# traveller59/spconv

Measured on AMD Instinct MI355X. Metric: active-voxels/sec fwd+bwd, 3x3x3 SubMConv3d C=64, ~100k voxels/scene, higher is better.
Workload: dtype f16; 1 GPU; SubMConv3d 3x3x3 C=64->64 f16, 100000 uniform voxels/scene in 1600x1280x40 (BASELINE configs[1]), 8 distinct scenes per GPU visited round-robin, rulebook reused via indice_key; voxels_per_gpu=100000, launch=hipgraph, steps_per_replay=8, scenes_rotated=8, mask_sort=False, prewarm_steps=0, parallelism=dp1, ranks_seen=1, tree=unknown

## Files before the change

spconv_amd/csrc/igemm_bwd.h:

```cpp
#pragma once
#include "igemm_v4.h"

namespace spx {
namespace {

constexpr int kWT = 64;

constexpr int kW2MaxG = 1024;
constexpr int kW2J = 128;
constexpr int kW2Rec = 8;
constexpr int kXcds = 8;


__host__ __device__ inline int plan2_wg(int w) { return 8 + kW2Rec * w; }
__host__ __device__ inline int plan2_kf(int G) { return 8 + kW2Rec * G; }
__host__ __device__ inline int plan2_seg(int G, int kv) { return 8 + kW2Rec * G + kv + 1; }
__host__ __device__ inline int plan2_red(int G, int kv) {
  return (plan2_seg(G, kv) + 3 * (G + kv) + 3) & ~3;
}

__device__ __forceinline__ int wtr_x(int row) { return ((row >> 1) & 1) | (((row >> 3) & 1) << 1); }
__device__ __forceinline__ int wtr_slot(int row, int sl) {
  return row * 128 + ((((sl >> 1) ^ wtr_x(row)) << 5) | ((sl & 1) << 4));
}

typedef short s16x4 __attribute__((ext_vector_type(4)));

__device__ __forceinline__ uint4 wtr_frag(const char *stage, int row0, int lrow, int gran) {
  const int r = row0 + (lrow >> 2);
  const char *a0 = stage + r * 128 + ((gran ^ wtr_x(r)) << 5) + ((lrow & 3) << 3);
  const int r1 = r + 4;
  const char *a1 = stage + r1 * 128 + ((gran ^ wtr_x(r1)) << 5) + ((lrow & 3) << 3);
  typedef __attribute__((address_space(3))) s16x4 lds_s16x4;
  const s16x4 lo = __builtin_amdgcn_ds_read_tr16_b64_v4i16(
      (lds_s16x4 *)(__attribute__((address_space(3))) char *)a0);
  const s16x4 hi = __builtin_amdgcn_ds_read_tr16_b64_v4i16(
      (lds_s16x4 *)(__attribute__((address_space(3))) char *)a1);
  const uint2 l2 = __builtin_bit_cast(uint2, lo), h2 = __builtin_bit_cast(uint2, hi);
  return make_uint4(l2.x, l2.y, h2.x, h2.y);
}

template <bool BF16, int STAGES, int SL = 8>
__device__ __forceinline__ void wgrad_tr_body(const Wgrad2Params &p, int block) {
  extern __shared__ __attribute__((aligned(16))) char smem[];
  constexpr int TILE_B = kW2J * 128;
  constexpr int RQ = SL / 2;
  constexpr int RSTEP = 2 * kW2J / SL;
  constexpr int RA = RQ < 2 ? 2 : RQ;
  const int tid = threadIdx.x, lane = tid & 63, wave = tid >> 6;
  const int lrow = lane & 15, lgrp = lane >> 4;
  const int wk = wave >> 1, wc = wave & 1;
  const int ntile = p.tiles_k * p.tiles_c;
  const int wb = block / ntile, tile = block - wb * ntile;
  const int w = p.xcd_order ? p.plan2[plan2_wg(wb) + 5] : wb;
  const int kk0 = (tile / p.tiles_c) * kWT, c0 = (tile % p.tiles_c) * kWT;
  const int32_t *__restrict__ rec = p.plan2 + plan2_wg(w);
  const int32_t *__restrict__ segs = p.plan2 + plan2_seg(p.G, p.kv);
  const int seg_lo = rec[0], nseg = rec[1];
  const bool live = kk0 + wk * 32 < p.K && c0 + wc * 32 < p.C;
  SPX_STAMP(0);

  const uint32_t rowD = static_cast<uint32_t>(p.K) * 2u, rowF = static_cast<uint32_t>(p.C) * 2u;
  const __amdgpu_buffer_rsrc_t rD = make_rsrc(p.dout, static_cast<uint32_t>(p.n_out) * rowD);
  const __amdgpu_buffer_rsrc_t rF = make_rsrc(p.feat, static_cast<uint32_t>(p.n_in) * rowF);
  const uint32_t list_bytes = (static_cast<uint32_t>(p.kv) + 1u) * static_cast<uint32_t>(p.n_in) * 4u;
  const uint32_t out_list = static_cast<uint32_t>(p.kv) * static_cast<uint32_t>(p.n_in) * 4u;

  const int slot = tid & (SL - 1), r0 = tid / SL;
  const uint32_t dcol = kk0 + slot * 8 < p.K ? static_cast<uint32_t>(kk0 + slot * 8) * 2u : kOob;
  const uint32_t fcol = c0 + slot * 8 < p.C ? static_cast<uint32_t>(c0 + slot * 8) * 2u : kOob;
  constexpr int W_ROWS = 64 / SL;
  const int wl_idx = lane & 31;
  const int wl_row = (64 * wave) / SL + (wl_idx % W_ROWS) + RSTEP * (wl_idx / W_ROWS);
  const uint32_t wl_list = (lane >> 5) ? out_list : 0u;
  const int rsub = lane / SL;
  int lds_w[RA];
#pragma unroll
  for (int q = 0; q < RQ; ++q) lds_w[q] = wtr_slot(r0 + RSTEP * q, slot);
  if constexpr (SL < 8) {
    for (int o = tid * 16; o < STAGES * 2 * TILE_B; o += kThreads * 16)
      *reinterpret_cast<u32x4 *>(smem + o) = u32x4{0u, 0u, 0u, 0u};
    __syncthreads();
  }

  for (int si = 0; si < nseg; ++si) {
    int k, begin, end;
    if (si == 0) {
      k = rec[2];
      begin = rec[3];
      end = rec[4];
    } else {
      k = segs[3 * (seg_lo + si)];
      begin = segs[3 * (seg_lo + si) + 1];
      end = segs[3 * (seg_lo + si) + 2];
    }
    const bool identity = p.subm && k == p.kv / 2;
    const __amdgpu_buffer_rsrc_t rW = make_rsrc(p.native + static_cast<size_t>(k) * p.n_in, list_bytes);

    f32x4 acc[2][2];
#pragma unroll
    for (int a = 0; a < 2; ++a)
#pragma unroll
      for (int b = 0; b < 2; ++b) acc[a][b] = f32x4{0.f, 0.f, 0.f, 0.f};

    uint32_t wd = 0;
    u32x4 dv[RA], fv[RA];
    auto load_words = [&](int base) __attribute__((always_inline)) {
      const int j = base + wl_row;
      if (identity) {
        wd = static_cast<uint32_t>(j);
      } else {
        const uint32_t vo = j < end ? static_cast<uint32_t>(j) * 4u + wl_list : kOob;
        wd = __builtin_amdgcn_raw_buffer_load_b32(rW, vo, 0, SPX_AUX_TABLE);
      }
    };
    auto load_rows = [&](int base) __attribute__((always_inline)) {
#pragma unroll
      for (int q = 0; q < RQ; ++q) {
        const uint32_t iq = static_cast<uint32_t>(
            __builtin_amdgcn_ds_bpermute((q * W_ROWS + rsub) * 4, static_cast<int>(wd)));
        const uint32_t oq = static_cast<uint32_t>(
            __builtin_amdgcn_ds_bpermute((32 + q * W_ROWS + rsub) * 4, static_cast<int>(wd)));
        const bool ok = base + r0 + RSTEP * q < end;
        dv[q] = __builtin_amdgcn_raw_buffer_load_b128(rD, ok ? (oq * rowD + dcol) | (dcol & kOob) : kOob, 0, 0);
        fv[q] = __builtin_amdgcn_raw_buffer_load_b128(rF, ok ? (iq * rowF + fcol) | (fcol & kOob) : kOob, 0, 0);
      }
    };
    load_words(begin);
    load_rows(begin);
    load_words(begin + kW2J);
    if (si == 0) SPX_STAMP(1);
    int stage = 0;
    for (int base = begin; base < end; base += kW2J, stage ^= (STAGES - 1)) {
      char *sD = smem + stage * (2 * TILE_B);
      char *sF = sD + TILE_B;
      if (STAGES == 1) __syncthreads();
#pragma unroll
      for (int q = 0; q < RQ; ++q) {
        *reinterpret_cast<u32x4 *>(sD + lds_w[q]) = dv[q];
        *reinterpret_cast<u32x4 *>(sF + lds_w[q]) = fv[q];
      }
      __syncthreads();
      load_rows(base + kW2J);
      load_words(base + 2 * kW2J);
      if (live)
#pragma unroll
      for (int ks = 0; ks < kW2J / 32; ++ks) {
        const int row0 = ks * 32 + lgrp * 8;
        uint4 fa[2], fb[2];
#pragma unroll
        for (int a = 0; a < 2; ++a) fa[a] = wtr_frag(sD, row0, lrow, wk * 2 + a);
#pragma unroll
        for (int b = 0; b < 2; ++b) fb[b] = wtr_frag(sF, row0, lrow, wc * 2 + b);
#pragma unroll
        for (int a = 0; a < 2; ++a)
#pragma unroll
          for (int b = 0; b < 2; ++b) acc[a][b] = mfma16<BF16>(fa[a], fb[b], acc[a][b]);
      }
    }
    if (si == nseg - 1) SPX_STAMP(4);
    float *dst = p.partial + (static_cast<size_t>(seg_lo + si) * ntile + tile) * (kWT * kWT);
#pragma unroll
    for (int a = 0; a < 2; ++a)
#pragma unroll
      for (int b = 0; b < 2; ++b)
#pragma unroll
        for (int e = 0; e < 4; ++e) {
          const int kk = wk * 32 + a * 16 + lgrp * 4 + e;
          const int c = wc * 32 + b * 16 + lrow;
          if (SPX_AUX_OUT) __builtin_nontemporal_store(acc[a][b][e], &dst[kk * kWT + c]);
          else dst[kk * kWT + c] = acc[a][b][e];
        }
    __syncthreads();
  }
  SPX_STAMP(6);
#ifdef SPX_TIMELINE
  asm volatile("s_waitcnt vmcnt(0)" ::: "memory");
  SPX_STAMP(7);
#endif
}

constexpr int kW3J = 64;
constexpr int kW3Stride = 80;

__device__ __forceinline__ void wgrad_f32_body(const Wgrad2Params &p, int block) {
  extern __shared__ __attribute__((aligned(16))) char smem[];
  float *sD = reinterpret_cast<float *>(smem);
  float *sF = sD + kW3J * kW3Stride;
  const int tid = threadIdx.x, lane = tid & 63, wave = tid >> 6;
  const int lrow = lane & 15, lgrp = lane >> 4;
  const int wk = wave >> 1, wc = wave & 1;
  const int ntile = p.tiles_k * p.tiles_c;
  const int w = block / ntile, tile = block - w * ntile;
  const int kk0 = (tile / p.tiles_c) * kWT, c0 = (tile % p.tiles_c) * kWT;
  const int32_t *__restrict__ rec = p.plan2 + plan2_wg(w);
  const int32_t *__restrict__ segs = p.plan2 + plan2_seg(p.G, p.kv);
  const int seg_lo = rec[0], nseg = rec[1];
  const uint32_t rowD = static_cast<uint32_t>(p.K) * 4u, rowF = static_cast<uint32_t>(p.C) * 4u;
  const __amdgpu_buffer_rsrc_t rD = make_rsrc(p.dout, static_cast<uint32_t>(p.n_out) * rowD);
  const __amdgpu_buffer_rsrc_t rF = make_rsrc(p.feat, static_cast<uint32_t>(p.n_in) * rowF);
  const uint32_t list_bytes = static_cast<uint32_t>(p.n_in) * 4u;
  const int slot = tid & 15, r0 = tid >> 4;
  const uint32_t dcol = kk0 + slot * 4 < p.K ? static_cast<uint32_t>(kk0 + slot * 4) * 4u : kOob;
  const uint32_t fcol = c0 + slot * 4 < p.C ? static_cast<uint32_t>(c0 + slot * 4) * 4u : kOob;

  for (int si = 0; si < nseg; ++si) {
    int k, begin, end;
    if (si == 0) {
      k = rec[2];
      begin = rec[3];
      end = rec[4];
    } else {
      k = segs[3 * (seg_lo + si)];
      begin = segs[3 * (seg_lo + si) + 1];
      end = segs[3 * (seg_lo + si) + 2];
    }
    const bool identity = p.subm && k == p.kv / 2;
    const __amdgpu_buffer_rsrc_t rIn =
        make_rsrc(p.native + static_cast<size_t>(k) * p.n_in, list_bytes);
    const __amdgpu_buffer_rsrc_t rOut =
        make_rsrc(p.native + static_cast<size_t>(p.kv + k) * p.n_in, list_bytes);
    f32x4 acc[2][2];
#pragma unroll
    for (int a = 0; a < 2; ++a)
#pragma unroll
      for (int b = 0; b < 2; ++b) acc[a][b] = f32x4{0.f, 0.f, 0.f, 0.f};
    u32x4 dv[4], fv[4];
    auto load_rows = [&](int base) __attribute__((always_inline)) {
#pragma unroll
      for (int q = 0; q < 4; ++q) {
        const int j = base + r0 + 16 * q;
        const bool ok = j < end;
        uint32_t ii = static_cast<uint32_t>(j), oi = static_cast<uint32_t>(j);
        if (!identity) {
          const uint32_t vo = ok ? static_cast<uint32_t>(j) * 4u : kOob;
          ii = __builtin_amdgcn_raw_buffer_load_b32(rIn, vo, 0, 0);
          oi = __builtin_amdgcn_raw_buffer_load_b32(rOut, vo, 0, 0);
        }
        dv[q] = __builtin_amdgcn_raw_buffer_load_b128(rD, ok ? (oi * rowD + dcol) | (dcol & kOob) : kOob, 0, 0);
        fv[q] = __builtin_amdgcn_raw_buffer_load_b128(rF, ok ? (ii * rowF + fcol) | (fcol & kOob) : kOob, 0, 0);
      }
    };
    load_rows(begin);
    for (int base = begin; base < end; base += kW3J) {
      __syncthreads();
#pragma unroll
      for (int q = 0; q < 4; ++q) {
        *reinterpret_cast<u32x4 *>(sD + (r0 + 16 * q) * kW3Stride + slot * 4) = dv[q];
        *reinterpret_cast<u32x4 *>(sF + (r0 + 16 * q) * kW3Stride + slot * 4) = fv[q];
      }
      __syncthreads();
      load_rows(base + kW3J);
#pragma unroll 4
      for (int ks = 0; ks < kW3J / 4; ++ks) {
        const int row = (ks * 4 + lgrp) * kW3Stride;
        float fa[2], fb[2];
#pragma unroll
        for (int a = 0; a < 2; ++a) fa[a] = sD[row + wk * 32 + a * 16 + lrow];
#pragma unroll
        for (int b = 0; b < 2; ++b) fb[b] = sF[row + wc * 32 + b * 16 + lrow];
#pragma unroll
        for (int a = 0; a < 2; ++a)
#pragma unroll
          for (int b = 0; b < 2; ++b)
            acc[a][b] = __builtin_amdgcn_mfma_f32_16x16x4f32(fa[a], fb[b], acc[a][b], 0, 0, 0);
      }
    }
    float *dst = p.partial + (static_cast<size_t>(seg_lo + si) * ntile + tile) * (kWT * kWT);
#pragma unroll
    for (int a = 0; a < 2; ++a)
#pragma unroll
      for (int b = 0; b < 2; ++b)
#pragma unroll
        for (int e = 0; e < 4; ++e) {
          const int kk = wk * 32 + a * 16 + lgrp * 4 + e;
          const int c = wc * 32 + b * 16 + lrow;
          if (SPX_AUX_OUT) __builtin_nontemporal_store(acc[a][b][e], &dst[kk * kWT + c]);
          else dst[kk * kWT + c] = acc[a][b][e];
        }
    __syncthreads();
  }
}

template <int COUT, int MB, int DT, int NKS = 2, int PK = 1>
__global__ void __launch_bounds__(kThreads, COUT <= 64 ? 4 : 2)
igemm_bwd_kernel(const void *argA, const void *argB, const uint32_t *arg_mask,
                 const int32_t *arg_argsort, const int32_t *arg_pair, int n_dst, int n_src, int CIN,
                 int kv, int identity_k, int b_reverse, GemmRest rest, int n_dgrad, Wgrad2Params wp) {
  const int nw = n_dgrad < 0 ? ~n_dgrad : 0;
  const int b = static_cast<int>(blockIdx.x);
  const bool is_dgrad = n_dgrad < 0 ? b >= nw : b < n_dgrad;
  if (is_dgrad) {
    GemmParams p;
    unpack_gemm_args(p, argA, argB, arg_mask, arg_argsort, arg_pair, n_dst, n_src, CIN, kv,
                     identity_k, b_reverse, rest);
    p.xcd_rot = (rest.dbg & 0x100) ? 0 : (nw & 7);
    p.app_budget = kAppBudget;
    igemm_v4_body<COUT, MB, DT, true, NKS, PK>(p, n_dgrad < 0 ? b - nw : b);
  } else {
    if constexpr (DT == 3) wgrad_f32_body(wp, n_dgrad < 0 ? b : b - n_dgrad);
    else wgrad_tr_body<DT == 1, 1>(wp, n_dgrad < 0 ? b : b - n_dgrad);
  }
}

template <int COUT, int MB, int DT = 0>
constexpr size_t bwd_smem_bytes() {
  const size_t a = v4_smem_bytes<COUT, MB>();
  const size_t b = DT == 3 ? 2 * static_cast<size_t>(kW3J) * kW3Stride * sizeof(float)
                           : 2 * static_cast<size_t>(kW2J) * 128;
  return a > b ? a : b;
}

template <int COUT, int MB, int DT>
int launch_bwd(const GemmParams &p, const Wgrad2Params &q, int n_wgrad_blocks, hipStream_t s) {
  const int napp = p.cls ? layout_app_tiles(p.n_dst, 64 * MB) : 0;
  const int n_dgrad = div_up(p.n_dst, 64 * MB) + napp;
  GemmRest rr = rest_of(p);
  rr.napp = p.cls ? napp : -1;
  constexpr int wgrad_first = 1;
  GemmParams pl = p;
  pl.lpt = p.tile_order && n_dgrad + n_wgrad_blocks > 1024;
  count_launch(kFamBwdFused);
#define SPX_LAUNCH_BWD(NKSV, PKV)                                                                                  \
  do {                                                                                                               \
    count_inst<inst::bwd(COUT, MB, DT, NKSV, PKV)>();                                                                \
    hipLaunchKernelGGL((igemm_bwd_kernel<COUT, MB, DT, NKSV, PKV>), dim3(n_dgrad + n_wgrad_blocks), dim3(kThreads),  \
                       (bwd_smem_bytes<COUT, MB, DT>()), s, p.A, p.B, p.mask, p.argsort, p.pair, p.n_dst,           \
                       p.n_src, p.CIN, p.kv, p.identity_k, v4_flags(pl), rr,                                        \
                       wgrad_first ? ~n_wgrad_blocks : n_dgrad, q);                                                 \
  } while (0)
  const int pk = v4_pack(p, DT, DT == 3 ? 4 : 2, true);
  if constexpr (DT == 0 || DT == 1) {
    if (pk == 32) SPX_LAUNCH_BWD(2, 32);
    else if (pk == 16) SPX_LAUNCH_BWD(2, 16);
    else if (pk == 8) SPX_LAUNCH_BWD(2, 8);
    else if (pk == 4) SPX_LAUNCH_BWD(1, 4);
    else if (pk == 2) SPX_LAUNCH_BWD(1, 2);
    else if (p.CIN * 2 <= 64) SPX_LAUNCH_BWD(1, 1);
    else SPX_LAUNCH_BWD(2, 1);
  } else {
    if (p.CIN * (DT == 3 ? 4 : 2) <= 64) SPX_LAUNCH_BWD(1, 1);
    else SPX_LAUNCH_BWD(2, 1);
  }
#undef SPX_LAUNCH_BWD
  SPX_LAUNCH_CHECK();
  return 0;
}

template <int DT>
int dispatch_bwd(const GemmParams &p, const Wgrad2Params &q, int nwb, hipStream_t s) {
  switch (p.COUT) {
    case 16: return launch_bwd<16, 2, DT>(p, q, nwb, s);
    case 32: return launch_bwd<32, 2, DT>(p, q, nwb, s);
    case 64: return launch_bwd<64, 2, DT>(p, q, nwb, s);
    case 128: return launch_bwd<128, 2, DT>(p, q, nwb, s);
  }
  return -1;
}

}
}
```

spconv_amd/csrc/igemm_wgrad.hip:

```cpp
#include <cstring>
#include "igemm_bwd.h"

namespace spx {
namespace {

constexpr int kWJ = 128;

struct WgradParams {
  const void *feat;
  const void *dout;
  float *partial;
  const int32_t *native;
  const int32_t *num;
  const int32_t *plan;
  int n_in, n_out, C, K, kv, subm, chunk, nchunks, tiles_c, tiles_k;
};

__device__ __forceinline__ int list_count(const int32_t *num, int kv, int subm, int n_in, int k) {
  int c;
  if (!subm) c = num[k];
  else if (k == kv / 2) c = n_in;
  else c = k < kv / 2 ? num[k] : num[kv - 1 - k];
  return c < n_in ? c : n_in;
}
// ... 102 lines not shown
          const int sh = (e & 1) * 16;
          const uint32_t dd = ((dword_of(dv[q][0], e >> 1) >> sh) & 0xffffu) |
                              (((dword_of(dv[q][1], e >> 1) >> sh) & 0xffffu) << 16);
          const uint32_t ff = ((dword_of(fv[q][0], e >> 1) >> sh) & 0xffffu) |
                              (((dword_of(fv[q][1], e >> 1) >> sh) & 0xffffu) << 16);
          const int col = wswz(ch, j);
          *reinterpret_cast<uint32_t *>(ldsD + ch * kWJ + col) = dd;
          *reinterpret_cast<uint32_t *>(ldsF + ch * kWJ + col) = ff;
        }
      }
      __syncthreads();
      if (base + kWJ < end) load_rows(base + kWJ);
#pragma unroll
      for (int ks = 0; ks < kWJ / 32; ++ks) {
        const int j8 = (ks * 4 + (lane >> 4)) * 8;
        uint4 fa[2], fb[2];
#pragma unroll
        for (int a = 0; a < 2; ++a) {
          const int ch = wk * 32 + a * 16 + (lane & 15);
          fa[a] = *reinterpret_cast<const uint4 *>(ldsD + ch * kWJ + wswz(ch, j8));
        }
#pragma unroll
        for (int b = 0; b < 2; ++b) {
          const int ch = wc * 32 + b * 16 + (lane & 15);
          fb[b] = *reinterpret_cast<const uint4 *>(ldsF + ch * kWJ + wswz(ch, j8));
        }
#pragma unroll
        for (int a = 0; a < 2; ++a)
#pragma unroll
          for (int b = 0; b < 2; ++b) acc[a][b] = mfma16<BF16>(fa[a], fb[b], acc[a][b]);
      }
    }
    float *dst = p.partial + static_cast<size_t>(work) * (kWT * kWT);
#pragma unroll
    for (int a = 0; a < 2; ++a)
#pragma unroll
      for (int b = 0; b < 2; ++b)
#pragma unroll
        for (int e = 0; e < 4; ++e) {
          const int kk = wk * 32 + a * 16 + (lane >> 4) * 4 + e;
          const int c = wc * 32 + b * 16 + (lane & 15);
          if (SPX_AUX_OUT) __builtin_nontemporal_store(acc[a][b][e], &dst[kk * kWT + c]);
          else dst[kk * kWT + c] = acc[a][b][e];
        }
    __syncthreads();
  }
}

template <typename T>
__global__ void __launch_bounds__(kThreads)
wgrad_generic_kernel(WgradParams p) {
  const int ntile = p.tiles_k * p.tiles_c;
  const int total = p.plan[0] * ntile;
  const int32_t *items = p.plan + 1 + 2 * p.kv;
  const T *F = static_cast<const T *>(p.feat);
  const T *D = static_cast<const T *>(p.dout);
  for (int work = blockIdx.x; work < total; work += gridDim.x) {
    const int item = work / ntile, tile = work - item * ntile;
    const int k = items[2 * item], begin = items[2 * item + 1];
    const int kk0 = (tile / p.tiles_c) * kWT, c0 = (tile % p.tiles_c) * kWT;
    const int cnt = list_count(p.num, p.kv, p.subm, p.n_in, k);
    const int end = min(cnt, begin + p.chunk);
    const bool identity = p.subm && k == p.kv / 2;
    const int32_t *in_list = p.native + static_cast<size_t>(k) * p.n_in;
    const int32_t *out_list = p.native + static_cast<size_t>(p.kv + k) * p.n_in;
    float *dst = p.partial + static_cast<size_t>(work) * (kWT * kWT);
    for (int e = threadIdx.x; e < kWT * kWT; e += kThreads) {
      const int kk = kk0 + e / kWT, c = c0 + e % kWT;
      float acc = 0.f;
      if (kk < p.K && c < p.C) {
        for (int j = begin; j < end; ++j) {
          const int oi = identity ? j : out_list[j];
          const int ii = identity ? j : in_list[j];
          acc = fmaf(load_f(D + static_cast<size_t>(oi) * p.K + kk),
                     load_f(F + static_cast<size_t>(ii) * p.C + c), acc);
        }
      }
      dst[e] = acc;
    }
  }
}

constexpr int kRedThreads = 512;
constexpr int kRedSplit = 16;
constexpr int kRedElems = kRedThreads / kRedSplit;

template <typename T>
__global__ void __launch_bounds__(kRedThreads)
wgrad_reduce_kernel(WgradParams p, T *__restrict__ dw) {
  __shared__ float red[kRedThreads];
  const int k = blockIdx.y;
  const int first = p.plan[1 + k], nch = p.plan[1 + p.kv + k];
  const int grp = threadIdx.x / kRedElems, el = threadIdx.x % kRedElems;
  const int ntile = p.tiles_k * p.tiles_c;
  const int e_global = blockIdx.x * kRedElems + el;
  const int tile = e_global / (kWT * kWT), e = e_global % (kWT * kWT);
  const size_t stride = static_cast<size_t>(ntile) * (kWT * kWT);
  float acc = 0.f;
  if (tile < ntile) {
    const float *src = p.partial + (static_cast<size_t>(first) * ntile + tile) * (kWT * kWT) + e;
    int ch = grp;
    for (; ch + 7 * kRedSplit < nch; ch += 8 * kRedSplit) {
      float v[8];
#pragma unroll
      for (int u = 0; u < 8; ++u) v[u] = src[static_cast<size_t>(ch + u * kRedSplit) * stride];
#pragma unroll
      for (int u = 0; u < 8; ++u) acc += v[u];
    }
    for (; ch < nch; ch += kRedSplit) acc += src[static_cast<size_t>(ch) * stride];
  }
  red[threadIdx.x] = acc;
  __syncthreads();
  if (grp == 0 && tile < ntile) {
    float s = 0.f;
#pragma unroll
    for (int g = 0; g < kRedSplit; ++g) s += red[g * kRedElems + el];
    const int kk = (tile / p.tiles_c) * kWT + e / kWT, c = (tile % p.tiles_c) * kWT + e % kWT;
    if (kk < p.K && c < p.C) store_f(dw + (static_cast<size_t>(kk) * p.kv + k) * p.C + c, s);
  }
}

template <typename T>
__device__ __forceinline__ T plan_scan(T v, T *wtot, T &total) {
  const int tid = threadIdx.x, lane = tid & 63, wv = tid >> 6;
  T incl = v;
#pragma unroll
  for (int d = 1; d < 64; d <<= 1) {
    const T u = __shfl_up(incl, d, 64);
    if (lane >= d) incl += u;
  }
  if (lane == 63) wtot[wv] = incl;
  __syncthreads();
  T prefix = 0;
  total = 0;
#pragma unroll
  for (int w = 0; w < kW2MaxG / 64; ++w) {
    const T t = wtot[w];
    if (w < wv) prefix += t;
    total += t;
  }
  return prefix + incl - v;
}

__device__ __forceinline__ bool subm_cost_pad(int n_in, int kv) {
  (void)n_in;
  (void)kv;
#ifdef SPX_WGRAD_NO_PAD
  return false;
#else
  return true;
#endif
}

__global__ void __launch_bounds__(kW2MaxG)
wgrad_plan2_kernel(const int32_t *__restrict__ num, int n_in, int kv, int subm, int G,
                   int32_t *__restrict__ plan) {
  typedef unsigned long long u64;
  __shared__ int start[130], lpad[130], kfirst[130], kcount[130], ritems[130];
  __shared__ int wtot_i[kW2MaxG / 64];
  __shared__ u64 wtot_a[kW2MaxG / 64], wtot_b[kW2MaxG / 64];
  const int tid = threadIdx.x;
  const int c = tid < kv ? list_count(num, kv, subm, n_in, tid) : 0;
  const int ov = (c > 0 && subm_cost_pad(n_in, kv)) ? kW2J + kW2J / 2 : 0;
  int total;
  const int st = plan_scan<int>(c + ov, wtot_i, total);
  if (tid <= kv) start[tid] = st;
  if (tid < kv) lpad[tid] = ov;
  const int per = total > 0 ? (total + G - 1) / G : 1;
  __syncthreads();
  auto pairs_in = [&](int k, int a, int b, int &pa, int &pb) {
    const int p0 = start[k] + lpad[k], len = start[k + 1] - p0;
    pa = min(max(a - p0, 0), len);
    pb = min(max(b - p0, 0), len);
  };

  int lo = 0, hi = 0, mine = 0, k0 = 0, x = 0;
  if (tid < G) {
    lo = min(total, tid * per);
    hi = min(total, lo + per);
    if (hi > lo) {
      int a = 0, b = kv;
      while (a < b) {
        const int m = (a + b) >> 1;
        if (start[m + 1] > lo) b = m;
        else a = m + 1;
      }
      k0 = a;
      for (int k = k0; k < kv && start[k] < hi; ++k) {
        int pa, pb;
        pairs_in(k, lo, hi, pa, pb);
        mine += pb > pa ? 1 : 0;
      }
      int pa, pb;
      pairs_in(k0, lo, hi, pa, pb);
      const int len = start[k0 + 1] - start[k0] - lpad[k0];
      x = min(kXcds - 1, static_cast<int>(static_cast<long long>(pa) * kXcds / (len > 0 ? len : 1)));
    }
  }
  int kc = 0, nitems = 0;
  if (tid < kv) {
    if (c > 0) kc = (start[tid + 1] - 1) / per - (start[tid] + ov) / per + 1;
    const int mode = kc >= 48 ? 0 : (kc >= 6 ? 1 : 2);
    nitems = (kWT * kWT) / (mode == 0 ? 16 : (mode == 1 ? 128 : 512));
  }
  u64 va = 0, vb = 0;
  if (tid < G) {
    va = static_cast<u64>(mine);
    if (x < 5) va |= 1ull << (11 + 10 * x);
    else vb = 1ull << (10 * (x - 5));
  }
  vb |= (static_cast<u64>(kc) << 30) | (static_cast<u64>(nitems) << 41);
  u64 ta, tb;
  const u64 ea = plan_scan<u64>(va, wtot_a, ta);
  const u64 eb = plan_scan<u64>(vb, wtot_b, tb);
  const int seg0 = static_cast<int>(ea & 0x7ff), nseg_total = static_cast<int>(ta & 0x7ff);
  const int kf = static_cast<int>((eb >> 30) & 0x7ff), ri = static_cast<int>(eb >> 41);
  const int kc_total = static_cast<int>((tb >> 30) & 0x7ff), items_total = static_cast<int>(tb >> 41);
  if (tid == 0) {
    plan[0] = nseg_total;
    plan[1] = per;
    plan[plan2_red(G, kv)] = items_total;
  }
  if (tid <= kv) {
    kfirst[tid] = kf;
    kcount[tid] = kc;
    ritems[tid] = ri;
    plan[plan2_kf(G) + tid] = tid == kv ? kc_total : kf;
  }
  int32_t *seg = plan + plan2_seg(G, kv);
  if (tid < G) {
    int sg = seg0;
    int32_t *rec = plan + plan2_wg(tid);
    int r2 = 0, r3 = 0, r4 = 0;
    bool first = true;
    if (hi > lo) {
      for (int k = k0; k < kv && start[k] < hi; ++k) {
        int a, b;
        pairs_in(k, lo, hi, a, b);
        if (b > a) {
          seg[3 * sg] = k;
          seg[3 * sg + 1] = a;
          seg[3 * sg + 2] = b;
          if (first) {
            r2 = k;
            r3 = a;
            r4 = b;
            first = false;
          }
          ++sg;
        }
      }
    }
    rec[0] = seg0;
    rec[1] = mine;
    rec[2] = r2;
    rec[3] = r3;
    rec[4] = r4;
    int pos = x < 5 ? static_cast<int>((ea >> (11 + 10 * x)) & 0x3ff) : static_cast<int>((eb >> (10 * (x - 5))) & 0x3ff);
#pragma unroll
    for (int y = 0; y < kXcds; ++y) {
      const int cy = y < 5 ? static_cast<int>((ta >> (11 + 10 * y)) & 0x3ff) : static_cast<int>((tb >> (10 * (y - 5))) & 0x3ff);
      if (y < x) pos += cy;
    }
    int y = 0, base = 0;
    for (; y < kXcds - 1; ++y) {
      const int ny = (G - y + kXcds - 1) / kXcds;
      if (pos < base + ny) break;
      base += ny;
    }
    const int b = y + kXcds * (pos - base);
    plan[plan2_wg(b < G ? b : tid) + 5] = tid;
  }
  __syncthreads();
  int32_t *rl = plan + plan2_red(G, kv);
  for (int k = 0; k < kv; ++k) {
    const int md = kcount[k] >= 48 ? 0 : (kcount[k] >= 6 ? 1 : 2);
    const int E = md == 0 ? 16 : (md == 1 ? 128 : 512), cnt_items = (kWT * kWT) / E;
    for (int q = tid; q < cnt_items; q += kW2MaxG) {
      int32_t *item = rl + 4 + 4 * (ritems[k] + q);
      item[0] = k | (md << 8);
      item[1] = q * E;
      item[2] = kfirst[k];
      item[3] = kcount[k];
    }
  }
}


template <bool BF16, int SL = 8>
__global__ void __launch_bounds__(kThreads)
wgrad_tr_kernel(Wgrad2Params p) {
  wgrad_tr_body<BF16, 2, SL>(p, blockIdx.x);
}


__global__ void __launch_bounds__(kThreads)
wgrad_f32_kernel(Wgrad2Params p) {
  wgrad_f32_body(p, blockIdx.x);
}


struct Wgrad2Job {
  const float *partial;
  const int32_t *plan2;
  void *dw;
  int G, kv, tiles_k, tiles_c, K, C;
};

template <typename T>
__device__ __forceinline__ void wgrad_reduce2_body(const Wgrad2Job &p, T *__restrict__ dw, const int tile, float *red) {
  const int32_t *__restrict__ rl = p.plan2 + plan2_red(p.G, p.kv);
  const int nitems = rl[0];
  const int ntile = p.tiles_k * p.tiles_c;
  const size_t stride = static_cast<size_t>(ntile) * (kWT * kWT);
  for (int it = blockIdx.x; it < nitems; it += gridDim.x) {
    const int4 item = *reinterpret_cast<const int4 *>(rl + 4 + 4 * it);
    const int k = item.x & 0xff, mode = item.x >> 8, e0 = item.y, first = item.z, nseg = item.w;
    const float *base = p.partial + static_cast<size_t>(first) * stride + tile * (kWT * kWT) + e0;
    if (mode == 0) {
      const int lane = threadIdx.x & 63, wave = threadIdx.x >> 6;
      const int c4 = lane & 3, grp = wave * 16 + (lane >> 2);
      float4 acc = make_float4(0.f, 0.f, 0.f, 0.f);
      const float *src = base + c4 * 4;
      int ch = grp;
      for (; ch + 3 * 128 < nseg; ch += 4 * 128) {
        float4 v[4];
#pragma unroll
        for (int u = 0; u < 4; ++u)
          v[u] = *reinterpret_cast<const float4 *>(src + static_cast<size_t>(ch + u * 128) * stride);
#pragma unroll
        for (int u = 0; u < 4; ++u) {
          acc.x += v[u].x; acc.y += v[u].y; acc.z += v[u].z; acc.w += v[u].w;
        }
      }
      for (; ch < nseg; ch += 128) {
        const float4 v = *reinterpret_cast<const float4 *>(src + static_cast<size_t>(ch) * stride);
        acc.x += v.x; acc.y += v.y; acc.z += v.z; acc.w += v.w;
      }
#pragma unroll
      for (int d = 4; d < 64; d <<= 1) {
        acc.x += __shfl_xor(acc.x, d, 64);
        acc.y += __shfl_xor(acc.y, d, 64);
        acc.z += __shfl_xor(acc.z, d, 64);
        acc.w += __shfl_xor(acc.w, d, 64);
      }
      if (lane < 4) reinterpret_cast<float4 *>(red)[wave * 4 + lane] = acc;
      __syncthreads();
      if (threadIdx.x < 16) {
        float sum = 0.f;
#pragma unroll
        for (int w = 0; w < kRedThreads / 64; ++w) sum += red[w * 16 + threadIdx.x];
        const int ee = e0 + threadIdx.x;
        const int kk = (tile / p.tiles_c) * kWT + ee / kWT, c = (tile % p.tiles_c) * kWT + ee % kWT;
        if (kk < p.K && c < p.C) store_f(dw + (static_cast<size_t>(kk) * p.kv + k) * p.C + c, sum);
      }
      __syncthreads();
      continue;
    }
    const int E = mode == 1 ? 128 : 512, S = kRedThreads / E;
    const int grp = threadIdx.x / E, el = threadIdx.x % E;
    float acc = 0.f;
    for (int ch = grp; ch < nseg; ch += S) acc += base[static_cast<size_t>(ch) * stride + el];
    if (S > 1) {
      red[threadIdx.x] = acc;
      __syncthreads();
      if (grp == 0) {
        acc = 0.f;
        for (int g = 0; g < S; ++g) acc += red[g * E + el];
      }
    }
    if (grp == 0) {
      const int ee = e0 + el;
      const int kk = (tile / p.tiles_c) * kWT + ee / kWT, c = (tile % p.tiles_c) * kWT + ee % kWT;
      if (kk < p.K && c < p.C) store_f(dw + (static_cast<size_t>(kk) * p.kv + k) * p.C + c, acc);
    }
    if (S > 1) __syncthreads();
  }
}


template <typename T>
__global__ void __launch_bounds__(kRedThreads)
wgrad_reduce2_kernel(Wgrad2Params p, T *__restrict__ dw) {
  __shared__ float red[kRedThreads];
  const Wgrad2Job j{p.partial, p.plan2, dw, p.G, p.kv, p.tiles_k, p.tiles_c, p.K, p.C};
  wgrad_reduce2_body<T>(j, dw, static_cast<int>(blockIdx.y), red);
}

constexpr int kStage2MaxJobs = 16;
struct Wgrad2Batch {
  int n;
  int ybase[kStage2MaxJobs + 1];
  Wgrad2Job job[kStage2MaxJobs];
};

template <typename T>
__global__ void __launch_bounds__(kRedThreads)
wgrad_reduce2_batch_kernel(Wgrad2Batch b) {
  __shared__ float red[kRedThreads];
  int j = 0;
  while (j + 1 < b.n && static_cast<int>(blockIdx.y) >= b.ybase[j + 1]) ++j;
  const Wgrad2Job job = b.job[j];
  wgrad_reduce2_body<T>(job, static_cast<T *>(job.dw), static_cast<int>(blockIdx.y) - b.ybase[j], red);
}

int wgrad_chunk(int n_in) {
  int c = (n_in / 512 + kWJ - 1) / kWJ * kWJ;
  if (c < kWJ) c = kWJ;
  if (c > 1024) c = 1024;
  return c;
}

size_t wgrad_plan_ints(int n_in, int kv) {
  const size_t nchunks = div_up(n_in > 0 ? n_in : 1, wgrad_chunk(n_in));
  return 1 + 2 * static_cast<size_t>(kv) + 2 * nchunks * kv;
}

int wgrad_groups(int n_in, int subm) {
  int g = 384;
  const int room = 1024 - div_up(n_in > 0 ? n_in : 1, 128) - ((subm && n_in >= kLayoutMinRows) ? kAppBudget : 0);
  if (room >= 128 && room < g) g = room;
  const int chunks = div_up(n_in > 0 ? n_in : 1, 128);
  if (g > 2 * chunks) g = 2 * chunks;
  if (g > kW2MaxG - 1) g = kW2MaxG - 1;
  return g < 1 ? 1 : g;
}

int wgrad_groups_max(int n_in) {
  const int a = wgrad_groups(n_in, 0), b = wgrad_groups(n_in, 1);
  return a > b ? a : b;
}

size_t wgrad_plan2_ints(int n_in, int kv) {
  const size_t G = wgrad_groups_max(n_in);
  return 8 + kW2Rec * G + kv + 1 + 3 * (G + kv) + 4 + 4 + 4 * static_cast<size_t>(kv) * 256 + 8;
}

size_t plan1_bytes(int n_in, int kv) {
  return align_up(wgrad_plan_ints(n_in, kv) * sizeof(int32_t), 256);
}

int reduce2_blocks(int kv) {
  constexpr int cap = 512;
  return kv * 256 < cap ? kv * 256 : cap;
}

struct Stage2JobH {
  const float *partial;
  const int32_t *plan2;
  void *dw;
  int G, kv, tiles_k, tiles_c, K, C, dtype, valid;
};
static_assert(sizeof(Stage2JobH) <= SPX_STAGE2_JOB_BYTES, "job record");

}

const int32_t *wgrad_plan_or_build(const int32_t *plan, const int32_t *num_per_loc, int n_in, int kv, int subm, void *ws,
                                   size_t ws_bytes, spx_stream_t stream) {
  if (plan) return plan;
  int32_t *own = reinterpret_cast<int32_t *>(static_cast<char *>(ws) + ws_bytes - spx_wgrad_plan_bytes(n_in, kv));
  return spx_wgrad_plan(num_per_loc, n_in, kv, subm, own, stream) ? nullptr : own;
}

Wgrad2Params wgrad2_params(const void *feat, const void *dout, void *ws, const int32_t *pair_native,
                           const int32_t *num_per_loc, const int32_t *plan, int n_in, int n_out, int C, int K, int kv,
                           int subm) {
  Wgrad2Params q{};
  q.feat = feat;
  q.dout = dout;
  q.partial = static_cast<float *>(ws);
  q.native = pair_native;
  q.num = num_per_loc;
  q.plan2 = reinterpret_cast<const int32_t *>(reinterpret_cast<const char *>(plan) + plan1_bytes(n_in, kv));
  q.n_in = n_in;
  q.n_out = n_out;
  q.C = C;
  q.K = K;
  q.kv = kv;
  q.subm = subm;
  q.tiles_c = div_up(C, kWT);
  q.tiles_k = div_up(K, kWT);
  q.G = wgrad_groups(n_in, subm);
  q.xcd_order = 1;
  return q;
}

int launch_reduce2(const Wgrad2Params &q, void *dw, int dtype, int ntile, hipStream_t s, void *defer) {
  if (defer) {
    Stage2JobH j{q.partial, q.plan2, dw, q.G, q.kv, q.tiles_k, q.tiles_c, q.K, q.C, dtype, 1};
    memcpy(defer, &j, sizeof(j));
    return 0;
  }
  const dim3 rgrid2(reduce2_blocks(q.kv), ntile);
  count_launch(kFamStage2);
  if (int rc = with_elem_type(dtype, [&](auto t, auto) {
        using T = decltype(t);
        hipLaunchKernelGGL(wgrad_reduce2_kernel<T>, rgrid2, dim3(kRedThreads), 0, s, q, static_cast<T *>(dw));
      }))
    return rc;
  SPX_LAUNCH_CHECK();
  return 0;
}

int igemm_wgrad_impl(const void *feat, const void *dout, void *dw, const int32_t *pair_native,
                     const int32_t *num_per_loc, const int32_t *plan, int n_in, int n_out, int C, int K, int kv,
                     int dtype, int subm, void *ws, size_t ws_bytes, spx_stream_t stream, void *stage2_job) {
  hipStream_t s = static_cast<hipStream_t>(stream);
  SPX_CHECK(dw && C > 0 && K > 0, "null tensor pointer");
  if (dtype == SPX_F64) {
    SPX_CHECK(kv >= 1, "bad kernel volume %d", kv);
    SPX_CHECK(!stage2_job, "float64 weight gradients have no deferred second stage");
    if (n_in == 0 || n_out == 0) {
      SPX_HIP(hipMemsetAsync(dw, 0, static_cast<size_t>(K) * kv * C * elem_bytes(dtype), s));
      return 0;
    }
    return wgrad_f64(feat, dout, dw, pair_native, num_per_loc, n_in, C, K, kv, subm, ws, ws_bytes, s);
  }
  SPX_CHECK(kv >= 1 && kv <= 128, "kernel volume %d not supported by wgrad (max 128)", kv);
  if (n_in == 0 || n_out == 0) {
    SPX_HIP(hipMemsetAsync(dw, 0, static_cast<size_t>(K) * kv * C * elem_bytes(dtype), s));
    return 0;
  }
  SPX_CHECK(feat && dout && ws, "null tensor pointer");
  SPX_CHECK(pair_native && num_per_loc, "Native pair lists and counts are required");
  SPX_CHECK(ws_bytes >= spx_igemm_wgrad_ws_bytes(n_in, C, K, kv), "workspace too small");
  plan = wgrad_plan_or_build(plan, num_per_loc, n_in, kv, subm, ws, ws_bytes, stream);
  if (!plan) return -2;
  const bool mfma = (dtype == SPX_F16 || dtype == SPX_BF16) && C % 8 == 0 && K % 8 == 0;
  const bool tr_path = mfma && wgrad_rows_fit(n_in, n_out, C, K, 2) && wgrad_lists_fit(n_in, kv);
  const bool f32_path = dtype == SPX_F32 && C % 4 == 0 && K % 4 == 0 && wgrad_rows_fit(n_in, n_out, C, K, 4) &&
                        wgrad_f32_list_fits(n_in);
  if (f32_path || tr_path) {
    const Wgrad2Params q = wgrad2_params(feat, dout, ws, pair_native, num_per_loc, plan, n_in, n_out, C, K, kv, subm);
    const int ntile = q.tiles_c * q.tiles_k;
    const dim3 grid(static_cast<unsigned>(q.G) * ntile);
    const size_t lds = 2 * 2 * kW2J * 128;
    const int sl = (C <= 16 && K <= 16) ? 2 : ((C <= 32 && K <= 32) ? 4 : 8);
#define SPX_WGRAD_TR(BF, SL)                                                                 \
  do {                                                                                       \
    count_inst<inst::wgrad_tr(BF ? 1 : 0, SL)>();                                            \
    hipLaunchKernelGGL((wgrad_tr_kernel<BF, SL>), grid, dim3(kThreads), lds, s, q);          \
  } while (0)
    if (dtype == SPX_F32) {
      count_inst<inst::kWgradF32>();
      hipLaunchKernelGGL(wgrad_f32_kernel, grid, dim3(kThreads), 2 * kW3J * kW3Stride * sizeof(float), s, q);
    } else if (dtype == SPX_F16) {
      if (sl == 2) SPX_WGRAD_TR(false, 2);
      else if (sl == 4) SPX_WGRAD_TR(false, 4);
      else SPX_WGRAD_TR(false, 8);
    } else {
      if (sl == 2) SPX_WGRAD_TR(true, 2);
      else if (sl == 4) SPX_WGRAD_TR(true, 4);
      else SPX_WGRAD_TR(true, 8);
    }
#undef SPX_WGRAD_TR
    return launch_reduce2(q, dw, dtype, ntile, s, stage2_job);
  }
  int32_t *plan1 = reinterpret_cast<int32_t *>(static_cast<char *>(ws) + ws_bytes - spx_wgrad_plan_bytes(n_in, kv));
  hipLaunchKernelGGL(wgrad_plan_kernel, dim3(1), dim3(kThreads), 0, s, num_per_loc, n_in, kv, subm, wgrad_chunk(n_in),
                     plan1);
  WgradParams p{};
  p.feat = feat;
  p.dout = dout;
  p.partial = static_cast<float *>(ws);
  p.native = pair_native;
  p.num = num_per_loc;
  p.plan = plan1;
  p.n_in = n_in;
  p.n_out = n_out;
  p.C = C;
  p.K = K;
  p.kv = kv;
  p.subm = subm;
  p.chunk = wgrad_chunk(n_in);
  p.nchunks = div_up(n_in > 0 ? n_in : 1, p.chunk);
  p.tiles_c = div_up(C, kWT);
  p.tiles_k = div_up(K, kWT);
  const int ntile = p.tiles_c * p.tiles_k;
  {
    const long long bound = static_cast<long long>(p.nchunks) * kv * ntile;
    constexpr int max_grid = 1024;
    const dim3 grid(static_cast<unsigned>(bound < max_grid ? bound : max_grid));
    const size_t lds = 2 * kWT * kWJ * 2;
    if (mfma && dtype == SPX_F16) {
      count_inst<inst::wgrad_mfma(0)>();
      hipLaunchKernelGGL(wgrad_mfma_kernel<false>, grid, dim3(kThreads), lds, s, p);
    } else if (mfma) {
      count_inst<inst::wgrad_mfma(1)>();
// ... 126 lines not shown
```

Baseline: 4.090 billion voxels/s.

## Derive wgrad segments and reduce items on device from compact per-offset plan header

The plan kernel now writes only a compact per-kernel-offset header (start, left pad, first segment, reduce item base) plus an XCD permutation, instead of materialising per-workgroup records, a segment list and a per-item reduce list. The wgrad and reduce kernels load that header into wave lanes and recompute their segments and reduce items on the fly with readlane/ballot bisection. This removes the serial per-item writes and the global segment traversal in the planning kernel and shrinks plan memory traffic, but adds lane-broadcast arithmetic to the hot kernels' prologue and per-segment loop.

```diff
diff --git a/spconv_amd/csrc/igemm_bwd.h b/spconv_amd/csrc/igemm_bwd.h
--- a/spconv_amd/csrc/igemm_bwd.h
+++ b/spconv_amd/csrc/igemm_bwd.h
@@ -8,15 +8,132 @@
 
 constexpr int kW2MaxG = 1024;
 constexpr int kW2J = 128;
-constexpr int kW2Rec = 8;
 constexpr int kXcds = 8;
 
-
-__host__ __device__ inline int plan2_wg(int w) { return 8 + kW2Rec * w; }
-__host__ __device__ inline int plan2_kf(int G) { return 8 + kW2Rec * G; }
-__host__ __device__ inline int plan2_seg(int G, int kv) { return 8 + kW2Rec * G + kv + 1; }
-__host__ __device__ inline int plan2_red(int G, int kv) {
-  return (plan2_seg(G, kv) + 3 * (G + kv) + 3) & ~3;
+constexpr int kW2Hdr = 16;
+__host__ __device__ inline int plan2_off(int k) { return kW2Hdr + 4 * k; }
+__host__ __device__ inline int plan2_perm(int kv) { return (plan2_off(kv + 1) + 15) & ~15; }
+
+template <class F>
+__host__ __device__ inline int plan_bisect(int kv, int v, F next) {
+  int a = 0, b = kv;
+  while (a < b) {
+    const int m = (a + b) >> 1;
+    if (next(m) > v) b = m;
+    else a = m + 1;
+  }
+  return a;
+}
+struct WgradSeg {
+  int k, begin, end;
+};
+struct WgradCut {
+  int lo, hi;
+  int k0;
+  int k;
+};
+
+template <class H>
+__host__ __device__ inline void wgrad_pairs_in(const H &h, int k, int a, int b, int &pa, int &pb) {
+  const int p0 = h.start(k) + h.lpad(k), len = h.start(k + 1) - p0;
+  const int da = a - p0 > 0 ? a - p0 : 0, db = b - p0 > 0 ? b - p0 : 0;
+  pa = da < len ? da : len;
+  pb = db < len ? db : len;
+}
+
+template <class H>
+__host__ __device__ inline WgradCut wgrad_cut_begin(const H &h, int kv, int w) {
+  const int total = h.start(kv), per = h.per();
+  WgradCut c;
+  c.lo = w * per < total ? w * per : total;
+  c.hi = c.lo + per < total ? c.lo + per : total;
+  c.k0 = c.k = c.hi > c.lo ? h.first_list(c.lo) : kv;
+  return c;
+}
+
+template <class H>
+__host__ __device__ inline bool wgrad_cut_next(const H &h, int kv, WgradCut &c, WgradSeg &s) {
+  for (; c.k < kv && h.start(c.k) < c.hi; ++c.k) {
+    int pa, pb;
+    wgrad_pairs_in(h, c.k, c.lo, c.hi, pa, pb);
+    if (pb > pa) {
+      s.k = c.k++;
+      s.begin = pa;
+      s.end = pb;
+      return true;
+    }
+  }
+  return false;
+}
+
+template <class H>
+__host__ __device__ inline int wgrad_seg_index(const H &h, int w, int k) {
+  return h.kfirst(k) + w - (h.start(k) + h.lpad(k)) / h.per();
+}
+
+__host__ __device__ inline int reduce2_mode(int nseg) { return nseg >= 48 ? 0 : (nseg >= 6 ? 1 : 2); }
+__host__ __device__ inline int reduce2_elems(int mode) { return mode == 0 ? 16 : (mode == 1 ? 128 : 512); }
+
+struct Reduce2Item {
+  int k, mode, e0, first, nseg;
+};
+template <class H>
+__host__ __device__ inline Reduce2Item reduce2_item(const H &h, int kv, int it) {
+  const int a = h.first_item_list(it);
+  Reduce2Item r;
+  r.k = a;
+  r.first = h.kfirst(a);
+  r.nseg = h.kfirst(a + 1) - r.first;
+  r.mode = reduce2_mode(r.nseg);
+  r.e0 = (it - h.ritems(a)) * reduce2_elems(r.mode);
+  return r;
+}
+
+template <int NEXT>
+struct PlanHdrLanes {
+  i32x4 v0, v1;
+  int n0, n1;
+  i32x4 s;
+  int kv;
+  __device__ __forceinline__ void settle() const {
+    const int all = v0[0] | v0[1] | v0[2] | v0[3] | v1[0] | v1[1] | v1[2] | v1[3] | n0 | n1;
+    asm volatile("" ::"s"(__builtin_amdgcn_readfirstlane(all)));
+  }
+  __device__ __forceinline__ int pick(int f, int k) const {
+    const int v = k < 64 ? v0[f] : v1[f];
+    return __builtin_amdgcn_readlane(v, k & 63);
+  }
+  __device__ __forceinline__ int per() const { return s[1]; }
+  __device__ __forceinline__ int start(int k) const { const int x = pick(0, k); return k >= 128 ? s[2] : x; }
+  __device__ __forceinline__ int lpad(int k) const { return pick(1, k); }
+  __device__ __forceinline__ int kfirst(int k) const { const int x = pick(2, k); return k >= 128 ? s[0] : x; }
+  __device__ __forceinline__ int ritems(int k) const { const int x = pick(3, k); return k >= 128 ? s[3] : x; }
+  __device__ __forceinline__ int count_le(int v) const {
+    const int lane = threadIdx.x & 63;
+    const unsigned long long m0 = __ballot(lane < kv && n0 <= v), m1 = __ballot(64 + lane < kv && n1 <= v);
+    return __builtin_popcountll(m0) + __builtin_popcountll(m1);
+  }
+  __device__ __forceinline__ int first_list(int v) const {
+    static_assert(NEXT == 0, "the lanes hold another field");
+    return count_le(v);
+  }
+  __device__ __forceinline__ int first_item_list(int v) const {
+    static_assert(NEXT == 3, "the lanes hold another field");
+    return count_le(v);
+  }
+};
+template <int NEXT>
+__device__ __forceinline__ PlanHdrLanes<NEXT> plan_hdr_load(const int32_t *__restrict__ plan2, int kv) {
+  const int lane = threadIdx.x & 63;
+  const __amdgpu_buffer_rsrc_t r = make_rsrc(plan2 + kW2Hdr, (static_cast<uint32_t>(kv) + 1u) * 16u);
+  PlanHdrLanes<NEXT> h;
+  h.v0 = __builtin_bit_cast(i32x4, __builtin_amdgcn_raw_buffer_load_b128(r, lane * 16, 0, 0));
+  h.v1 = __builtin_bit_cast(i32x4, __builtin_amdgcn_raw_buffer_load_b128(r, (64 + lane) * 16, 0, 0));
+  h.n0 = static_cast<int>(__builtin_amdgcn_raw_buffer_load_b32(r, (lane + 1) * 16 + NEXT * 4, 0, 0));
+  h.n1 = static_cast<int>(__builtin_amdgcn_raw_buffer_load_b32(r, (65 + lane) * 16 + NEXT * 4, 0, 0));
+  h.s = *reinterpret_cast<const i32x4 *>(plan2);
+  h.kv = kv;
+  return h;
 }
 
 __device__ __forceinline__ int wtr_x(int row) { return ((row >> 1) & 1) | (((row >> 3) & 1) << 1); }
@@ -52,11 +169,9 @@
   const int wk = wave >> 1, wc = wave & 1;
   const int ntile = p.tiles_k * p.tiles_c;
   const int wb = block / ntile, tile = block - wb * ntile;
-  const int w = p.xcd_order ? p.plan2[plan2_wg(wb) + 5] : wb;
+  const int w = p.xcd_order ? p.plan2[plan2_perm(p.kv) + wb] : wb;
+  const PlanHdrLanes<0> hdr = plan_hdr_load<0>(p.plan2, p.kv);
   const int kk0 = (tile / p.tiles_c) * kWT, c0 = (tile % p.tiles_c) * kWT;
-  const int32_t *__restrict__ rec = p.plan2 + plan2_wg(w);
-  const int32_t *__restrict__ segs = p.plan2 + plan2_seg(p.G, p.kv);
-  const int seg_lo = rec[0], nseg = rec[1];
   const bool live = kk0 + wk * 32 < p.K && c0 + wc * 32 < p.C;
   SPX_STAMP(0);
 
@@ -83,17 +198,13 @@
     __syncthreads();
   }
 
-  for (int si = 0; si < nseg; ++si) {
-    int k, begin, end;
-    if (si == 0) {
-      k = rec[2];
-      begin = rec[3];
-      end = rec[4];
-    } else {
-      k = segs[3 * (seg_lo + si)];
-      begin = segs[3 * (seg_lo + si) + 1];
-      end = segs[3 * (seg_lo + si) + 2];
-    }
+  hdr.settle();
+  WgradCut cut = wgrad_cut_begin(hdr, p.kv, w);
+  WgradSeg sg;
+  bool first_seg = true;
+  bool more = wgrad_cut_next(hdr, p.kv, cut, sg);
+  while (more) {
+    const int k = sg.k, begin = sg.begin, end = sg.end;
     const bool identity = p.subm && k == p.kv / 2;
     const __amdgpu_buffer_rsrc_t rW = make_rsrc(p.native + static_cast<size_t>(k) * p.n_in, list_bytes);
 
@@ -129,7 +240,10 @@
     load_words(begin);
     load_rows(begin);
     load_words(begin + kW2J);
-    if (si == 0) SPX_STAMP(1);
+    if (first_seg) SPX_STAMP(1);
+    first_seg = false;
+    const int seg = wgrad_seg_index(hdr, w, k);
+    more = wgrad_cut_next(hdr, p.kv, cut, sg);
     int stage = 0;
     for (int base = begin; base < end; base += kW2J, stage ^= (STAGES - 1)) {
       char *sD = smem + stage * (2 * TILE_B);
@@ -158,8 +272,8 @@
           for (int b = 0; b < 2; ++b) acc[a][b] = mfma16<BF16>(fa[a], fb[b], acc[a][b]);
       }
     }
-    if (si == nseg - 1) SPX_STAMP(4);
-    float *dst = p.partial + (static_cast<size_t>(seg_lo + si) * ntile + tile) * (kWT * kWT);
+    SPX_STAMP(4);
+    float *dst = p.partial + (static_cast<size_t>(seg) * ntile + tile) * (kWT * kWT);
 #pragma unroll
     for (int a = 0; a < 2; ++a)
 #pragma unroll
@@ -193,9 +307,7 @@
   const int ntile = p.tiles_k * p.tiles_c;
   const int w = block / ntile, tile = block - w * ntile;
   const int kk0 = (tile / p.tiles_c) * kWT, c0 = (tile % p.tiles_c) * kWT;
-  const int32_t *__restrict__ rec = p.plan2 + plan2_wg(w);
-  const int32_t *__restrict__ segs = p.plan2 + plan2_seg(p.G, p.kv);
-  const int seg_lo = rec[0], nseg = rec[1];
+  const PlanHdrLanes<0> hdr = plan_hdr_load<0>(p.plan2, p.kv);
   const uint32_t rowD = static_cast<uint32_t>(p.K) * 4u, rowF = static_cast<uint32_t>(p.C) * 4u;
   const __amdgpu_buffer_rsrc_t rD = make_rsrc(p.dout, static_cast<uint32_t>(p.n_out) * rowD);
   const __amdgpu_buffer_rsrc_t rF = make_rsrc(p.feat, static_cast<uint32_t>(p.n_in) * rowF);
@@ -204,17 +316,12 @@
   const uint32_t dcol = kk0 + slot * 4 < p.K ? static_cast<uint32_t>(kk0 + slot * 4) * 4u : kOob;
   const uint32_t fcol = c0 + slot * 4 < p.C ? static_cast<uint32_t>(c0 + slot * 4) * 4u : kOob;
 
-  for (int si = 0; si < nseg; ++si) {
-    int k, begin, end;
-    if (si == 0) {
-      k = rec[2];
-      begin = rec[3];
-      end = rec[4];
-    } else {
-      k = segs[3 * (seg_lo + si)];
-      begin = segs[3 * (seg_lo + si) + 1];
-      end = segs[3 * (seg_lo + si) + 2];
-    }
+  hdr.settle();
+  WgradCut cut = wgrad_cut_begin(hdr, p.kv, w);
+  WgradSeg sg;
+  bool more = wgrad_cut_next(hdr, p.kv, cut, sg);
+  while (more) {
+    const int k = sg.k, begin = sg.begin, end = sg.end;
     const bool identity = p.subm && k == p.kv / 2;
     const __amdgpu_buffer_rsrc_t rIn =
         make_rsrc(p.native + static_cast<size_t>(k) * p.n_in, list_bytes);
@@ -242,6 +349,8 @@
       }
     };
     load_rows(begin);
+    const int seg = wgrad_seg_index(hdr, w, k);
+    more = wgrad_cut_next(hdr, p.kv, cut, sg);
     for (int base = begin; base < end; base += kW3J) {
       __syncthreads();
 #pragma unroll
@@ -266,7 +375,7 @@
             acc[a][b] = __builtin_amdgcn_mfma_f32_16x16x4f32(fa[a], fb[b], acc[a][b], 0, 0, 0);
       }
     }
-    float *dst = p.partial + (static_cast<size_t>(seg_lo + si) * ntile + tile) * (kWT * kWT);
+    float *dst = p.partial + (static_cast<size_t>(seg) * ntile + tile) * (kWT * kWT);
 #pragma unroll
     for (int a = 0; a < 2; ++a)
 #pragma unroll
diff --git a/spconv_amd/csrc/igemm_wgrad.hip b/spconv_amd/csrc/igemm_wgrad.hip
--- a/spconv_amd/csrc/igemm_wgrad.hip
+++ b/spconv_amd/csrc/igemm_wgrad.hip
@@ -278,11 +278,22 @@
 #endif
 }
 
+struct PlanHdrLds {
+  const int *st, *lp;
+  int per_, kv;
+  __device__ __forceinline__ int per() const { return per_; }
+  __device__ __forceinline__ int start(int k) const { return st[k]; }
+  __device__ __forceinline__ int lpad(int k) const { return lp[k]; }
+  __device__ __forceinline__ int first_list(int v) const {
+    return plan_bisect(kv, v, [this](int k) { return st[k + 1]; });
+  }
+};
+
 __global__ void __launch_bounds__(kW2MaxG)
 wgrad_plan2_kernel(const int32_t *__restrict__ num, int n_in, int kv, int subm, int G,
                    int32_t *__restrict__ plan) {
   typedef unsigned long long u64;
-  __shared__ int start[130], lpad[130], kfirst[130], kcount[130], ritems[130];
+  __shared__ int start[130], lpad[130];
   __shared__ int wtot_i[kW2MaxG / 64];
   __shared__ u64 wtot_a[kW2MaxG / 64], wtot_b[kW2MaxG / 64];
   const int tid = threadIdx.x;
@@ -291,34 +302,18 @@
   int total;
   const int st = plan_scan<int>(c + ov, wtot_i, total);
   if (tid <= kv) start[tid] = st;
-  if (tid < kv) lpad[tid] = ov;
+  if (tid <= kv) lpad[tid] = tid < kv ? ov : 0;
   const int per = total > 0 ? (total + G - 1) / G : 1;
   __syncthreads();
-  auto pairs_in = [&](int k, int a, int b, int &pa, int &pb) {
-    const int p0 = start[k] + lpad[k], len = start[k + 1] - p0;
-    pa = min(max(a - p0, 0), len);
-    pb = min(max(b - p0, 0), len);
-  };
-
-  int lo = 0, hi = 0, mine = 0, k0 = 0, x = 0;
+  const PlanHdrLds h{start, lpad, per, kv};
+
+  int x = 0;
   if (tid < G) {
-    lo = min(total, tid * per);
-    hi = min(total, lo + per);
-    if (hi > lo) {
-      int a = 0, b = kv;
-      while (a < b) {
-        const int m = (a + b) >> 1;
-        if (start[m + 1] > lo) b = m;
-        else a = m + 1;
-      }
-      k0 = a;
-      for (int k = k0; k < kv && start[k] < hi; ++k) {
-        int pa, pb;
-        pairs_in(k, lo, hi, pa, pb);
-        mine += pb > pa ? 1 : 0;
-      }
+    WgradCut cut = wgrad_cut_begin(h, kv, tid);
+    if (cut.hi > cut.lo) {
+      const int k0 = cut.k0;
       int pa, pb;
-      pairs_in(k0, lo, hi, pa, pb);
+      wgrad_pairs_in(h, k0, cut.lo, cut.hi, pa, pb);
       const int len = start[k0 + 1] - start[k0] - lpad[k0];
       x = min(kXcds - 1, static_cast<int>(static_cast<long long>(pa) * kXcds / (len > 0 ? len : 1)));
     }
@@ -326,62 +321,33 @@
   int kc = 0, nitems = 0;
   if (tid < kv) {
     if (c > 0) kc = (start[tid + 1] - 1) / per - (start[tid] + ov) / per + 1;
-    const int mode = kc >= 48 ? 0 : (kc >= 6 ? 1 : 2);
-    nitems = (kWT * kWT) / (mode == 0 ? 16 : (mode == 1 ? 128 : 512));
+    nitems = (kWT * kWT) / reduce2_elems(reduce2_mode(kc));
   }
   u64 va = 0, vb = 0;
   if (tid < G) {
-    va = static_cast<u64>(mine);
-    if (x < 5) va |= 1ull << (11 + 10 * x);
+    if (x < 5) va = 1ull << (11 + 10 * x);
     else vb = 1ull << (10 * (x - 5));
   }
   vb |= (static_cast<u64>(kc) << 30) | (static_cast<u64>(nitems) << 41);
   u64 ta, tb;
   const u64 ea = plan_scan<u64>(va, wtot_a, ta);
   const u64 eb = plan_scan<u64>(vb, wtot_b, tb);
-  const int seg0 = static_cast<int>(ea & 0x7ff), nseg_total = static_cast<int>(ta & 0x7ff);
   const int kf = static_cast<int>((eb >> 30) & 0x7ff), ri = static_cast<int>(eb >> 41);
-  const int kc_total = static_cast<int>((tb >> 30) & 0x7ff), items_total = static_cast<int>(tb >> 41);
+  const int items_total = static_cast<int>(tb >> 41);
   if (tid == 0) {
-    plan[0] = nseg_total;
+    plan[0] = static_cast<int>((tb >> 30) & 0x7ff);
     plan[1] = per;
-    plan[plan2_red(G, kv)] = items_total;
+    plan[2] = total;
+    plan[3] = items_total;
   }
   if (tid <= kv) {
-    kfirst[tid] = kf;
-    kcount[tid] = kc;
-    ritems[tid] = ri;
-    plan[plan2_kf(G) + tid] = tid == kv ? kc_total : kf;
-  }
-  int32_t *seg = plan + plan2_seg(G, kv);
+    int32_t *row = plan + plan2_off(tid);
+    row[0] = st;
+    row[1] = tid < kv ? ov : 0;
+    row[2] = kf;
+    row[3] = ri;
+  }
   if (tid < G) {
-    int sg = seg0;
-    int32_t *rec = plan + plan2_wg(tid);
-    int r2 = 0, r3 = 0, r4 = 0;
-    bool first = true;
-    if (hi > lo) {
-      for (int k = k0; k < kv && start[k] < hi; ++k) {
-        int a, b;
-        pairs_in(k, lo, hi, a, b);
-        if (b > a) {
-          seg[3 * sg] = k;
-          seg[3 * sg + 1] = a;
-          seg[3 * sg + 2] = b;
-          if (first) {
-            r2 = k;
-            r3 = a;
-            r4 = b;
-            first = false;
-          }
-          ++sg;
-        }
-      }
-    }
-    rec[0] = seg0;
-    rec[1] = mine;
-    rec[2] = r2;
-    rec[3] = r3;
-    rec[4] = r4;
     int pos = x < 5 ? static_cast<int>((ea >> (11 + 10 * x)) & 0x3ff) : static_cast<int>((eb >> (10 * (x - 5))) & 0x3ff);
 #pragma unroll
     for (int y = 0; y < kXcds; ++y) {
@@ -395,20 +361,7 @@
       base += ny;
     }
     const int b = y + kXcds * (pos - base);
-    plan[plan2_wg(b < G ? b : tid) + 5] = tid;
-  }
-  __syncthreads();
-  int32_t *rl = plan + plan2_red(G, kv);
-  for (int k = 0; k < kv; ++k) {
-    const int md = kcount[k] >= 48 ? 0 : (kcount[k] >= 6 ? 1 : 2);
-    const int E = md == 0 ? 16 : (md == 1 ? 128 : 512), cnt_items = (kWT * kWT) / E;
-    for (int q = tid; q < cnt_items; q += kW2MaxG) {
-      int32_t *item = rl + 4 + 4 * (ritems[k] + q);
-      item[0] = k | (md << 8);
-      item[1] = q * E;
-      item[2] = kfirst[k];
-      item[3] = kcount[k];
-    }
+    plan[plan2_perm(kv) + (b < G ? b : tid)] = tid;
   }
 }
 
@@ -435,13 +388,14 @@
 
 template <typename T>
 __device__ __forceinline__ void wgrad_reduce2_body(const Wgrad2Job &p, T *__restrict__ dw, const int tile, float *red) {
-  const int32_t *__restrict__ rl = p.plan2 + plan2_red(p.G, p.kv);
-  const int nitems = rl[0];
+  const PlanHdrLanes<3> hdr = plan_hdr_load<3>(p.plan2, p.kv);
+  hdr.settle();
+  const int nitems = hdr.ritems(p.kv);
   const int ntile = p.tiles_k * p.tiles_c;
   const size_t stride = static_cast<size_t>(ntile) * (kWT * kWT);
   for (int it = blockIdx.x; it < nitems; it += gridDim.x) {
-    const int4 item = *reinterpret_cast<const int4 *>(rl + 4 + 4 * it);
-    const int k = item.x & 0xff, mode = item.x >> 8, e0 = item.y, first = item.z, nseg = item.w;
+    const Reduce2Item item = reduce2_item(hdr, p.kv, it);
+    const int k = item.k, mode = item.mode, e0 = item.e0, first = item.first, nseg = item.nseg;
     const float *base = p.partial + static_cast<size_t>(first) * stride + tile * (kWT * kWT) + e0;
     if (mode == 0) {
       const int lane = threadIdx.x & 63, wave = threadIdx.x >> 6;
@@ -559,7 +513,8 @@
 
 size_t wgrad_plan2_ints(int n_in, int kv) {
   const size_t G = wgrad_groups_max(n_in);
-  return 8 + kW2Rec * G + kv + 1 + 3 * (G + kv) + 4 + 4 + 4 * static_cast<size_t>(kv) * 256 + 8;
+  const size_t need = plan2_perm(kv) + G, was = 8 + 8 * G + kv + 1 + 3 * (G + kv) + 4 + 4 + 4 * static_cast<size_t>(kv) * 256 + 8;
+  return need > was ? need : was;
 }
 
 size_t plan1_bytes(int n_in, int kv) {
```

New measurement: 4.126 billion voxels/s, median of 6. Within noise of the previous version (+0.9%).
